# PBozmarov/RL-Environment-for-Component-Placement

Measured on AMD Instinct MI355X. Metric: env_steps_per_sec, higher is better.
Workload: dtype u64; 1 GPU; c3: 64x64 grid, 16 components, 48 pins, reward=centroid; envs_per_gpu=4096, queue_depth=2, instances=replay, fresh_instance_every_reset=False, incremental_obs=False, loop=fused, store_policy=sc1 (write-through)

## Files before the change

### rl-environment-for-component-placement_amd/csrc/pcb_device.h

```cpp
#pragma once
#include <hip/hip_runtime.h>
#include <math.h>
#include <stdint.h>

#include <type_traits>

#include "pcb_records.h"

__device__ inline u64 load_agent(const u64 *p) { return __hip_atomic_load(p, __ATOMIC_RELAXED, __HIP_MEMORY_SCOPE_AGENT); }
__device__ inline unsigned load_agent(const unsigned *p) { return __hip_atomic_load(p, __ATOMIC_RELAXED, __HIP_MEMORY_SCOPE_AGENT); }
__device__ inline int load_agent(const int *p) { return __hip_atomic_load(p, __ATOMIC_RELAXED, __HIP_MEMORY_SCOPE_AGENT); }
__device__ inline void store_agent(unsigned *p, unsigned v) { __hip_atomic_store(p, v, __ATOMIC_RELAXED, __HIP_MEMORY_SCOPE_AGENT); }
#ifdef PCBENV_STAMPS
#define STAMP(k) do { if ((threadIdx.x & (NT - 1)) == 0 && p.dbg) { unsigned long long t_; asm volatile("s_memtime %0\n\ts_waitcnt lgkmcnt(0)" : "=s"(t_) :: "memory"); p.dbg[(size_t)blockIdx.x * 32 + (k)] = t_; } } while (0)
#define STAMP_RT(k) do { if ((threadIdx.x & (NT - 1)) == 0 && p.dbg) { unsigned long long t_; asm volatile("s_memrealtime %0\n\ts_waitcnt lgkmcnt(0)" : "=s"(t_) :: "memory"); p.dbg[(size_t)blockIdx.x * 32 + (k)] = t_; } } while (0)
#define STAMP_T0() unsigned long long st0_; asm volatile("s_memtime %0\n\ts_waitcnt lgkmcnt(0)" : "=s"(st0_) :: "memory")
#define STAMP_ACC_SINCE(k, dep) do { unsigned long long t_; asm volatile("s_memtime %0\n\ts_waitcnt lgkmcnt(0)" : "=s"(t_) : "v"(dep) : "memory"); if ((threadIdx.x & (NT - 1)) == 0 && p.dbg) p.dbg[(size_t)blockIdx.x * 32 + (k)] += t_ - st0_; } while (0)
#define STAMP_ADD(k, v) do { if ((threadIdx.x & (NT - 1)) == 0 && p.dbg) p.dbg[(size_t)blockIdx.x * 32 + (k)] += (unsigned long long)(v); } while (0)
#define STAMP_ZERO(k) do { if ((threadIdx.x & (NT - 1)) == 0 && p.dbg) p.dbg[(size_t)blockIdx.x * 32 + (k)] = 0ull; } while (0)
#define STAMP_ROWS_BY_ENV(launch, e) DevParams p = (launch); if (p.dbg) p.dbg += ((long long)(e) - (long long)blockIdx.x) * 32
#else
#define STAMP(k) do { } while (0)
#define STAMP_RT(k) do { } while (0)
#define STAMP_T0() do { } while (0)
#define STAMP_ACC_SINCE(k, dep) do { } while (0)
#define STAMP_ADD(k, v) do { } while (0)
#define STAMP_ZERO(k) do { } while (0)
#define STAMP_ROWS_BY_ENV(launch, e) const DevParams &p = (launch)
#endif


template <int WW> struct Row;
template <> struct Row<1> {
    u64 a;
    __device__ static Row load(const u64 *p) { return Row{p[0]}; }
    __device__ void store(u64 *p) const { p[0] = a; }
    __device__ Row operator|(Row o) const { return Row{a | o.a}; }
    __device__ Row shr(int k) const { return Row{k >= 64 ? 0ull : a >> k}; }
    __device__ static Row zero() { return Row{0ull}; }
    __device__ bool any() const { return a != 0; }
    __device__ Row free_below(int n) const { return Row{n <= 0 ? 0ull : (~a & (n >= 64 ? ~0ull : ((1ull << n) - 1ull)))}; }
};
template <> struct Row<2> {
    u64 a, b;
    __device__ static Row load(const u64 *p) { return Row{p[0], p[1]}; }
    __device__ void store(u64 *p) const { p[0] = a; p[1] = b; }
    __device__ Row operator|(Row o) const { return Row{a | o.a, b | o.b}; }
    __device__ Row shr(int k) const {
        if (k == 0) return *this;
        if (k >= 128) return Row{0ull, 0ull};
        if (k >= 64) return Row{b >> (k - 64), 0ull};
        return Row{(a >> k) | (b << (64 - k)), b >> k};
    }
    __device__ static Row zero() { return Row{0ull, 0ull}; }
    __device__ bool any() const { return (a | b) != 0; }
    __device__ Row free_below(int n) const {
        u64 ma = n <= 0 ? 0ull : (n >= 64 ? ~0ull : ((1ull << n) - 1ull));
        u64 mb = n <= 64 ? 0ull : (n >= 128 ? ~0ull : ((1ull << (n - 64)) - 1ull));
        return Row{~a & ma, ~b & mb};
    }
};

template <int WW> __device__ inline Row<WW> hfold(Row<WW> r, int pw) {
    Row<WW> f = r;
    int s = 1;
    while (2 * s <= pw) { f = f | f.shr(s); s *= 2; }
    if (s < pw) f = f | f.shr(pw - s);
    return f;
}

typedef unsigned v4u __attribute__((ext_vector_type(4)));
#if defined(PCBENV_STORE_PLAIN)
struct ObsDst { unsigned char *base; };
__device__ inline ObsDst obs_dst(unsigned char *base, long long) { return ObsDst{base}; }
template <bool STREAM> __device__ inline void STORE16(const ObsDst &d, unsigned off, uint4 v) { *(uint4 *)(d.base + off) = v; }
#else
struct ObsDst { __amdgpu_buffer_rsrc_t rsrc; };
__device__ inline ObsDst obs_dst(unsigned char *base, long long bytes) {
    const uintptr_t b = (uintptr_t)base;
    const unsigned lo = (unsigned)__builtin_amdgcn_readfirstlane((int)(unsigned)b), hi = (unsigned)__builtin_amdgcn_readfirstlane((int)(unsigned)(b >> 32));
    unsigned char *ub = (unsigned char *)(((uintptr_t)hi << 32) | lo);
    return ObsDst{__builtin_amdgcn_make_buffer_rsrc(ub, 0, __builtin_amdgcn_readfirstlane((int)bytes), 0x00020000)};
}
#define PCBENV_AUX_SC1 16
#define PCBENV_AUX_NT 2
template <bool STREAM> __device__ inline void STORE16(const ObsDst &d, unsigned off, uint4 v) {
    const v4u w{v.x, v.y, v.z, v.w};
    __builtin_amdgcn_raw_buffer_store_b128(w, d.rsrc, (int)off, 0, STREAM ? (PCBENV_AUX_SC1 | PCBENV_AUX_NT) : PCBENV_AUX_SC1);
}
#endif

__device__ inline unsigned expand4(unsigned b) { return (b * 0x00204081u) & 0x01010101u; }
__device__ inline uint4 expand16(unsigned bits) {
    return make_uint4(expand4(bits & 15u), expand4((bits >> 4) & 15u), expand4((bits >> 8) & 15u), expand4((bits >> 12) & 15u));
}

__device__ inline void STORE16_dyn(const ObsDst &d, unsigned off, uint4 v, bool stream) { if (stream) STORE16<true>(d, off, v); else STORE16<false>(d, off, v); }
__device__ inline u64 lane_down(u64 a, int s, int lane) {
    const int src = (lane + s) << 2;
    const unsigned lo = (unsigned)__builtin_amdgcn_ds_bpermute(src, (int)(unsigned)a), hi = (unsigned)__builtin_amdgcn_ds_bpermute(src, (int)(unsigned)(a >> 32));
    return lane + s < WAVE ? (((u64)hi << 32) | lo) : 0ull;
}
template <int G> __device__ inline int group_inclusive_scan(int x, int lane) {
    const int row = lane & 15;
    int t;
    t = __builtin_amdgcn_update_dpp(0, x, 0x111, 0xF, 0xF, false); if (row >= 1) x += t;
    t = __builtin_amdgcn_update_dpp(0, x, 0x112, 0xF, 0xF, false); if (row >= 2) x += t;
    t = __builtin_amdgcn_update_dpp(0, x, 0x114, 0xF, 0xF, false); if (row >= 4) x += t;
    t = __builtin_amdgcn_update_dpp(0, x, 0x118, 0xF, 0xF, false); if (row >= 8) x += t;
    if (G >= 32) { t = __builtin_amdgcn_update_dpp(0, x, 0x142, 0xF, 0xF, false); if ((lane & 31) >= 16) x += t; }
    if (G == 64) { t = __builtin_amdgcn_update_dpp(0, x, 0x143, 0xF, 0xF, false); if (lane >= 32) x += t; }
// ... 9 lines not shown
```

### rl-environment-for-component-placement_amd/csrc/pcb_kernels.h

```cpp
#pragma once
#include "pcb_team.h"
#include "pcb_launch.h"

template <int KIND, int WW, int NW>
__global__ __launch_bounds__(64 * NW) void k_reset(DevParams p, const unsigned char *__restrict__ mask) {
    typedef Team<64 * NW> T;
    extern __shared__ __attribute__((aligned(16))) unsigned char smem[];
    const int e = xcd_contiguous_env((int)blockIdx.x, 0, p.B), lane = threadIdx.x;
    if (mask && !mask[e]) return;
    T::load_state(smem, p, e, lane);
    Lds l = carve(smem, p);
    const int row = out_row(p, p.slot, e);
    T::template reset_env<KIND, WW, true>(p, l, e, row, lane);
    if (lane == 0) {
        l.hdr->pre_action = 0u;
        l.hdr->term_seq = 0u;
        p.buf.reward[row] = 0.0;
        p.buf.done[row] = 0;
        if (p.buf.info) { p.buf.info[2 * (size_t)row] = nan(""); p.buf.info[2 * (size_t)row + 1] = nan(""); }
    }
    T::store_state(smem, p, e, lane);
}

template <int KIND, int WW, int NW>
__global__ __launch_bounds__(64 * NW) void k_gather(DevParams p, GatherArgs g) {
    typedef Team<64 * NW> T;
    extern __shared__ __attribute__((aligned(16))) unsigned char smem[];
    const int e = xcd_contiguous_env((int)blockIdx.x, 0, p.B), lane = threadIdx.x;
    const int j = __builtin_amdgcn_readfirstlane(g.src_index[e]);
    const bool take = (unsigned)j < (unsigned)g.src_B;
    if (!take && j != -1 && g.errors && lane == 0) atomicOr(g.errors, 1u);
    const unsigned char *own = p.state + (size_t)e * p.stateStride;
    T::load_state_from(smem, take ? g.src_state + (size_t)j * p.stateStride : own, p, lane);
    Lds l = carve(smem, p);
    if (take) {
        if (lane == 0) {
            const EnvHdr *oh = (const EnvHdr *)own;
            l.hdr->qcursor = oh->qcursor; l.hdr->episode = oh->episode;
            l.hdr->term_seq = 0u; l.hdr->term_pos = 0u;
            l.hdr->pre_action = 0u;
            if (KIND == PCBENV_PIN || KIND == PCBENV_SPATIAL) l.hdr->feat_gen = p.bind_gen;
        }
        T::lds_sync();
        const int row = out_row(p, p.slot, e);
        if (KIND == PCBENV_SPATIAL) T::build_pin_tables(p, l, lane);
        T::template emit_features_full<KIND>(p, l, row, lane);
        if (KIND == PCBENV_SPATIAL) {
            T::emit_component_grid(p, l, row, lane);
            T::feat_cache_fill(p, l, e, lane);
            T::lds_sync();
        }
        T::template mask_and_emit<KIND, WW>(p, l, row, lane, true, 0, p.H);
        if (KIND == PCBENV_SPATIAL) T::template emit_pin_grid<WW>(p, l, row, lane, 0, p.H);
        if (lane == 0) {
            p.buf.reward[row] = g.reward[j];
            p.buf.done[row] = g.done[j];
            if (p.buf.info) {
                p.buf.info[2 * (size_t)row] = g.info ? g.info[2 * (size_t)j] : nan("");
                p.buf.info[2 * (size_t)row + 1] = g.info ? g.info[2 * (size_t)j + 1] : nan("");
            }
        }
    }
    T::store_state(smem, p, e, lane);
}

template <int KIND, int WW, int NW, bool ROUTES, int BUILD, int GEO = STEP_GEO_RUNTIME>
__global__ __attribute__((amdgpu_waves_per_eu(4, 8))) __launch_bounds__(64 * NW) void k_step(DevParams p, int *__restrict__ actions, int fmt, int sampled,
                                               u64 seed, u64 first_env, u64 step_index, int num_steps_) {
    extern __shared__ __attribute__((aligned(16))) unsigned char smem[];
    constexpr bool TRAJ = BUILD == STEP_BUILD_SLOT || BUILD == STEP_BUILD_ROLLOUT;
    if (!TRAJ) p.stream_stores = BUILD == STEP_BUILD_INPLACE_STREAM;
    if (GEO == STEP_GEO_64) {
        static_assert(GEO == STEP_GEO_RUNTIME || (pcb_layout::is_pin_kind(KIND) && WW == 1 && NW == 1 && !ROUTES && !TRAJ), "pcb_layout::fixed_geometry_applies");
        constexpr pcb_layout::FixedGeometry g = pcb_layout::fixed_geometry(KIND);
        p.H = g.H; p.W = g.W; p.O = g.O; p.WW = g.WW;
        p.offOcc = g.offOcc; p.offVm = g.offVm; p.offComps = g.offComps;
        p.buf.grid = (uint8_t *)((uintptr_t)p.buf.grid & ~(uintptr_t)15);
        p.buf.action_mask = (uint8_t *)((uintptr_t)p.buf.action_mask & ~(uintptr_t)15);
        p.buf.pin_grid = (uint8_t *)((uintptr_t)p.buf.pin_grid & ~(uintptr_t)15);
    }
    const int num_steps = BUILD == STEP_BUILD_ROLLOUT ? num_steps_ : 1;
    __builtin_amdgcn_s_setprio(3);
    constexpr bool HELPERS = KIND == PCBENV_PIN || KIND == PCBENV_SPATIAL;
    const int nh = HELPERS ? p.term_wgs * p.term_hpe : 0;
    int e = (int)blockIdx.x - nh, role = ROLE_ENV, part = 0;
    if (e >= 0) e = xcd_contiguous_env((int)blockIdx.x, nh, p.B);
    unsigned pos = 0u;
    if (HELPERS && e < 0) {
        const unsigned hb = blockIdx.x, hpe = (unsigned)p.term_hpe, k = hb / hpe;
        part = (int)(hb - k * hpe);
        const unsigned ring = p.seq & 3u, cps = (unsigned)p.term_cap / TERM_SHARDS, shard = k & (TERM_SHARDS - 1u), idx = k >> TERM_SHARD_BITS;
        const unsigned cnt = (unsigned)__builtin_amdgcn_readfirstlane((int)load_agent(p.term_cnt + (ring * TERM_SHARDS + shard) * TERM_CNT_STRIDE));
        if (idx >= cps || idx >= cnt) return;
        pos = k;
        e = __builtin_amdgcn_readfirstlane(p.term_list[ring * (unsigned)p.term_cap + pos]);
        if ((unsigned)e >= (unsigned)p.B) return;
        role = part < REWARD_PARTS ? ROLE_REWARD : ROLE_FEATURES;
    } else if (p.term_cap > 0 && e == 0 && threadIdx.x < TERM_SHARDS) {
        unsigned *hist = p.term_cnt + TERM_HIST_OFFSET;
        unsigned longest = load_agent(p.term_cnt + (((p.seq & 3u) * TERM_SHARDS + threadIdx.x) * TERM_CNT_STRIDE));
        const unsigned h1 = hist[(p.seq + 1u) & 3u], h2 = hist[(p.seq + 2u) & 3u], h3 = hist[(p.seq + 3u) & 3u], told = hist[4];
        for (int o = TERM_SHARDS / 2; o > 0; o >>= 1) longest = max(longest, (unsigned)__shfl_xor((int)longest, o, TERM_SHARDS));
        const unsigned least = min(min(longest, h1), min(h2, h3));
        store_agent(p.term_cnt + ((((p.seq + 2u) & 3u) * TERM_SHARDS + threadIdx.x) * TERM_CNT_STRIDE), 0u);
        if (threadIdx.x == 0) {
            hist[p.seq & 3u] = longest;
            if (least > told || least + (told >> 3) + 2u < told) {
                hist[4] = least;
                __hip_atomic_store(p.term_seen, least, __ATOMIC_RELAXED, __HIP_MEMORY_SCOPE_SYSTEM);
            }
        }
    }
    Team<64 * NW>::template run_env<KIND, WW, ROUTES, TRAJ>(p, smem, e, threadIdx.x, actions, fmt, sampled, seed, first_env, step_index,
                                                           num_steps, role, part, pos);
}
```

### rl-environment-for-component-placement_amd/csrc/pcb_observe.h

```cpp
static __device__ inline void load_state_from(unsigned char *smem, const unsigned char *block, const DevParams &p, int lane) {
    const uint4 *src = (const uint4 *)block;
    uint4 *dst = (uint4 *)smem;
    const int n = (int)(p.stateStride / 16);
    if (n <= NT) {
        if (lane < n) dst[lane] = src[lane];
    } else {
        uint4 t[4];
        #pragma unroll
        for (int k = 0; k < 4; k++) { const int i = lane + k * NT; t[k] = i < n ? src[i] : make_uint4(0, 0, 0, 0); }
        #pragma unroll
        for (int k = 0; k < 4; k++) { const int i = lane + k * NT; if (i < n) dst[i] = t[k]; }
        for (int i = lane + 4 * NT; i < n; i += NT) dst[i] = src[i];
    }
    lds_sync();
}
static __device__ inline void load_state(unsigned char *smem, const DevParams &p, int e, int lane) {
    load_state_from(smem, p.state + (size_t)e * p.stateStride, p, lane);
}
static __device__ inline void store_state(const unsigned char *smem, const DevParams &p, int e, int lane) {
    lds_sync();
    uint4 *dst = (uint4 *)(p.state_out + (size_t)e * p.stateStride);
    const uint4 *src = (const uint4 *)smem;
    for (int i = lane; i < (int)(p.stateStride / 16); i += NT) dst[i] = src[i];
}

template <int KIND, int WW> static __device__ inline void emit_marginals(const DevParams &p, Lds &l, int row, int lane) {
    if (!p.buf.mask_rows && !p.buf.mask_orientation) return;
    const int H = p.H, plane = H * WW, O = p.O;
    for (int i = lane; i < O * H; i += NT) {
        const int o = i / H, r = i - o * H;
        const u64 *bits = l.vm + (o & 1) * plane + r * WW;
        bool a = false;
        for (int w = 0; w < WW; w++) a |= bits[w] != 0;
        if (p.buf.mask_rows) p.buf.mask_rows[(size_t)row * O * H + i] = a ? 1 : 0;
    }
    if (p.buf.mask_orientation) {
        for (int o = (int)(lane / WAVE); o < O; o += NT / WAVE) {
            bool a = false;
            for (int i = (lane & 63); i < plane; i += WAVE) a |= l.vm[(o & 1) * plane + i] != 0;
            a = __any(a);
            if ((lane & 63) == 0) p.buf.mask_orientation[(size_t)row * O + o] = a ? 1 : 0;
        }
    }
}

template <int KIND, int WW>
static __device__ inline bool mask_and_emit(const DevParams &p, Lds &l, int row, int lane, bool emit, int gr0, int gr1) {
    const int H = p.H, W = p.W, HW = H * W, plane = H * WW;
    const int cur = l.hdr->cur;
    unsigned char *m = (emit && p.buf.action_mask) ? p.buf.action_mask + (size_t)row * p.O * HW : 0;
    if (emit && p.buf.grid) emit_plane<WW>(p.buf.grid + (size_t)row * HW, l.occ, gr0, gr1, W, lane, p.stream_stores);
    bool any = false;
    if (KIND == PCBENV_SQUARE) {
        any = window_mask<WW>(l.occ, l.hf, l.vm, H, W, p.component_n, p.component_n, lane, &l.hdr->flag);
        if (m) emit_plane<WW>(m, l.vm, 0, H, W, lane, p.stream_stores);
        if (emit) emit_marginals<KIND, WW>(p, l, row, lane);
        return any;
    }
    const bool four = (KIND == PCBENV_PIN || KIND == PCBENV_SPATIAL);
    if (cur >= 0) {
        const int h = l.comps[cur].h, w = l.comps[cur].w;
        any = window_mask<WW>(l.occ, l.hf, l.vm, H, W, h, w, lane, &l.hdr->flag);
        if (m) { if (four) emit_plane2<WW>(m, m + 2 * HW, l.vm, H, W, lane, p.stream_stores); else emit_plane<WW>(m, l.vm, 0, H, W, lane, p.stream_stores); }
        if (h == w) {
            for (int i = lane; i < plane; i += NT) l.vm[plane + i] = l.vm[i];
            lds_sync();
        } else {
            any |= window_mask<WW>(l.occ, l.hf, l.vm + plane, H, W, w, h, lane, &l.hdr->flag);
        }
    } else {
        for (int i = lane; i < 2 * plane; i += NT) l.vm[i] = 0ull;
        lds_sync();
        if (m) { if (four) emit_plane2<WW>(m, m + 2 * HW, l.vm, H, W, lane, p.stream_stores); else emit_plane<WW>(m, l.vm, 0, H, W, lane, p.stream_stores); }
    }
    if (m) { if (four) emit_plane2<WW>(m + HW, m + 3 * HW, l.vm + plane, H, W, lane, p.stream_stores); else emit_plane<WW>(m + HW, l.vm + plane, 0, H, W, lane, p.stream_stores); }
    if (emit) emit_marginals<KIND, WW>(p, l, row, lane);
    return any;
}

#define CLS_EMPTY 0x80u
template <int WW> static __device__ inline void emit_pin_grid(const DevParams &p, Lds &l, int row, int lane, int r0, int r1) {
    if (!p.buf.pin_grid) return;
    const int W = p.W, HW = p.H * W, K = p.K;
    const int c0 = r0 * W, c1 = r1 * W;
    unsigned char *dst = p.buf.pin_grid + (size_t)row * HW * K;
    const long long b0 = (long long)c0 * K, b1 = (long long)c1 * K;
    if ((W & 15) == 0) {
        const int sh = (W & (W - 1)) == 0 ? __ffs(W) - 1 : -1;
        for (int ch = c0 / 16 + lane; ch < c1 / 16; ch += NT) {
            const int cell = ch * 16, r = sh >= 0 ? cell >> sh : cell / W, c = cell - r * W;
            uint4 v = expand16((unsigned)(l.occ[r * WW + (c >> 6)] >> (c & 63)) & 0xFFFFu);
            v.x |= (v.x ^ 0x01010101u) << 7; v.y |= (v.y ^ 0x01010101u) << 7; v.z |= (v.z ^ 0x01010101u) << 7; v.w |= (v.w ^ 0x01010101u) << 7;
            *(uint4 *)(l.cls + cell) = v;
        }
    } else {
        for (int i = c0 + lane; i < c1; i += NT) {
            int r = i / W, c = i - r * W;
            l.cls[i] = (unsigned char)(((l.occ[r * WW + (c >> 6)] >> (c & 63)) & 1ull) ? 1u : CLS_EMPTY);
        }
    }
    lds_sync();
    for (int q = lane; q < l.hdr->npins; q += NT) {
        const PinRec pr = l.pins[q];
        if (pr.abs_x >= r0 && pr.abs_x < r1 && pr.abs_y >= 0) l.cls[pr.abs_x * W + pr.abs_y] = (unsigned char)(pr.net + 2);
    }
    lds_sync();
    if ((b0 & 15) == 0 && (b1 & 15) == 0 && (((uintptr_t)dst) & 15) == 0) {
        const ObsDst d = obs_dst(dst, b1);
        const int first = ((int)(b0 / 16) + lane) * 16, dcell = 16 * NT / K, drem = 16 * NT - dcell * K;
        auto chunks = [&](auto stream_tag, auto cells_tag) {
            constexpr int NC = decltype(cells_tag)::value;
            int cell0 = first / K, rem = first - cell0 * K;
            for (int c = (int)(b0 / 16) + lane; c < (int)(b1 / 16); c += NT) {
                const int bb = c * 16;
                int cell = cell0;
                const int rem_now = rem;
                cell0 += dcell; rem += drem;
                if (rem >= K) { rem -= K; cell0++; }
                unsigned ones = 0u;
                if (K >= 5) {
                    unsigned cl[NC];
                    #pragma unroll
                    for (int j = 0; j < NC; j++) cl[j] = cell + j < c1 ? (unsigned)l.cls[cell + j] : CLS_EMPTY;
                    const int rel = -rem_now - 1;
                    #pragma unroll
                    for (int j = 0; j < NC; j++) {
                        const unsigned off = (unsigned)(rel + j * K + (int)cl[j]);
                        ones |= off < 16u ? 1u << off : 0u;
                    }
                } else {
                    for (int base = bb - rem_now; base < bb + 16 && cell < c1; base += K, cell++) {
                        const unsigned off = (unsigned)(base + (int)l.cls[cell] - 1 - bb);
                        if (off < 16u) ones |= 1u << off;
                    }
// ... 205 lines not shown
            double v = 0.0;
            if (c < nc) {
                const CompRec cr = l.comps[c];
                if (k == 0) v = cr.h; else if (k == 1) v = cr.w; else if (k == 2) v = cr.px; else if (k == 3) v = cr.py;
                else if (k == 4) v = (double)(cr.h * cr.w) / p.area;
                else {
                    const unsigned id = KIND == PCBENV_SPATIAL ? t.pid[c * p.mp + k - 5] : 0xFFFFu;
                    v = id == 0xFFFFu ? -1.0 : (double)id;
                }
            }
            cf[i] = v;
            c += dc; k += dk;
            if (k >= p.F) { k -= p.F; c++; }
        }
    }
    if (p.buf.placement_mask) {
        double *pm = p.buf.placement_mask + (size_t)row * p.C;
        for (int c = lane; c < p.C; c += NT) {
            const bool placed = c < nc && l.comps[c].px >= 0;
            pm[c] = KIND == PCBENV_RECT ? (placed ? 1.0 : 0.0) : (c >= nc ? 0.0 : placed ? 2.0 : c == cur ? 3.0 : 1.0);
        }
    }
    if (KIND == PCBENV_RECT && p.buf.component_mask) {
        double *cm = p.buf.component_mask + (size_t)row * p.C;
        for (int c = lane; c < p.C; c += NT) cm[c] = c < nc ? 1.0 : 0.0;
    }
    if (KIND == PCBENV_PIN || KIND == PCBENV_SPATIAL) {
        double *fn = p.buf.all_pins_num_feature ? p.buf.all_pins_num_feature + (size_t)row * p.pinRows * 4 : 0;
        double *fc = p.buf.all_pins_cat_feature ? p.buf.all_pins_cat_feature + (size_t)row * p.pinRows * p.catW : 0;
        if (!fn && !fc) return;
        if (KIND == PCBENV_SPATIAL) {
            for (int r = np + lane; r < p.pinRows; r += NT) {
                if (fn) { fn[4 * r] = 0.0; fn[4 * r + 1] = 0.0; fn[4 * r + 2] = 0.0; fn[4 * r + 3] = 0.0; }
                if (fc) { const double v = r == p.pinRows - 1 ? -1.0 : 0.0; fc[2 * r] = v; fc[2 * r + 1] = v; }
            }
            for (int q = lane; q < np; q += NT) {
                const PinRec pr = l.pins[q];
                const int r = pr.id & PIN_ID_MASK;
                if (fn) { fn[4 * r] = pr.rel_x; fn[4 * r + 1] = pr.rel_y; fn[4 * r + 2] = pr.abs_x; fn[4 * r + 3] = pr.abs_y; }
                if (fc) { fc[2 * r] = pr.net; fc[2 * r + 1] = pr.comp; }
            }
        } else if (p.pinRows <= p.ldsHfWords * 64) {
            u64 *rowbits = l.hf;
            lds_sync();
            for (int i = lane; i < p.ldsHfWords; i += NT) rowbits[i] = 0ull;
            lds_sync();
            for (int q = lane; q < np; q += NT) {
                const PinRec pr = l.pins[q];
                const int r = pr.comp * p.mp + (pr.id & PIN_ID_MASK);
                atomicOr((unsigned long long *)&rowbits[r >> 6], 1ull << (r & 63));
            }
            lds_sync();
            for (int r = lane; r < p.pinRows; r += NT) {
                if ((rowbits[r >> 6] >> (r & 63)) & 1ull) continue;
                if (fn) { fn[4 * r] = 0.0; fn[4 * r + 1] = 0.0; fn[4 * r + 2] = 0.0; fn[4 * r + 3] = 0.0; }
                if (fc) fc[r] = 0.0;
            }
            for (int q = lane; q < np; q += NT) {
                const PinRec pr = l.pins[q];
                if (pr.id & PIN_LOSER) continue;
                const int r = pr.comp * p.mp + (pr.id & PIN_ID_MASK);
                if (fn) { fn[4 * r] = pr.rel_x; fn[4 * r + 1] = pr.rel_y; fn[4 * r + 2] = pr.abs_x; fn[4 * r + 3] = pr.abs_y; }
                if (fc) fc[r] = pr.net;
            }
            lds_sync();
        } else {
            for (int i = lane; i < p.pinRows * 4; i += NT) if (fn) fn[i] = 0.0;
            for (int i = lane; i < p.pinRows; i += NT) if (fc) fc[i] = 0.0;
            store_drain_sync();
            for (int q = lane; q < np; q += NT) {
                const PinRec pr = l.pins[q];
                if (pr.id & PIN_LOSER) continue;
                const int r = pr.comp * p.mp + (pr.id & PIN_ID_MASK);
                if (fn) { fn[4 * r] = pr.rel_x; fn[4 * r + 1] = pr.rel_y; fn[4 * r + 2] = pr.abs_x; fn[4 * r + 3] = pr.abs_y; }
                if (fc) fc[r] = pr.net;
            }
        }
    }
}

template <int KIND, bool ROUTES>
static __device__ __forceinline__ void terminal_reward(const DevParams &p, Lds &l, int row, int lane, int part, int nparts, unsigned pos) {
    const bool placed_all = l.hdr->cur < 0;
    double reward, wl, ni;
    if (!placed_all) {
        reward = -p.w_wl * (p.max_wl / p.wl_norm) - p.w_int * (p.max_int / p.int_norm);
        wl = p.max_wl; ni = p.max_int;
    } else {
        double wsum[2] = {0.0, 0.0}; int cnt[2] = {0, 0};
        if (!ROUTES) route_centroid(p, l.hdr, l.pins, l.seg, lane, part, nparts, &wsum[0], &cnt[0]);
        else route_beam_or_both(p, l.hdr, l.pins, l.seg, lane, part, nparts, wsum, cnt);
        if (nparts > 1) {
            if (lane != 0) return;
            static_assert(REWARD_PARTS < 256 && PCBENV_MAX_PINS * (PCBENV_MAX_PINS - 1) / 2 < (1 << 28), "`mine`: 8 bits of arrivals, 28 bits per count of segment pairs");
            const u64 mine = 1ull | ((u64)(unsigned)cnt[0] << 8) | ((u64)(unsigned)cnt[1] << 36);
            const u64 before = atomicAdd((unsigned long long *)(p.term_arrive + pos), (unsigned long long)mine);
            if ((int)(before & 0xFFull) != nparts - 1) return;
            const u64 total = before + mine;
            cnt[0] = (int)((total >> 8) & 0xFFFFFFFull); cnt[1] = (int)(total >> 36);
            __hip_atomic_store(p.term_arrive + pos, 0ull, __ATOMIC_RELAXED, __HIP_MEMORY_SCOPE_AGENT);
        }
        const int pick = (ROUTES && p.reward_type == PCBENV_REWARD_BOTH && cnt[1] < cnt[0]) ? 1 : 0;
        wl = wsum[pick] / p.wl_norm;
        ni = (double)cnt[pick] / p.int_norm;
        reward = -1 * (p.w_wl * wl + p.w_int * ni);
    }
    if (lane == 0) {
        p.buf.reward[row] = reward;
        if (p.buf.info) { p.buf.info[2 * (size_t)row] = wl; p.buf.info[2 * (size_t)row + 1] = ni; }
    }
}
```

### rl-environment-for-component-placement_amd/csrc/pcb_reset.h

```cpp
static __device__ inline void fetch_instance(const DevParams &p, unsigned qcursor, int e, int lane, InstRegs &ir) {
    const unsigned slot = qcursor % (unsigned)p.Q;
    const unsigned char *rec = p.queue + ((size_t)slot * p.B + e) * p.instStride;
    const int *ih = (const int *)rec;
    const u64 *crec = (const u64 *)(rec + 16), *prec = crec + p.C;
    ir.nc = load_agent(ih); ir.nn = load_agent(ih + 1); ir.np = load_agent(ih + 2);
    ir.comp = lane < p.C ? load_agent(crec + lane) : 0ull;
    #pragma unroll
    for (int r = 0; r < 4; r++) { const int q = lane + r * NT; ir.pin[r] = q < p.P ? load_agent(prec + q) : 0ull; }
}

#define RESET_STATE_MASKS 1
#define RESET_FEATURES 2
#define RESET_ALL 3
template <int KIND, int WW, bool TRAJ> static __device__ inline void reset_env(const DevParams &p, Lds &l, int e, int row, int lane, int what = RESET_ALL) {
    const int H = p.H, W = p.W, HW = H * W;
    const bool owner = what & RESET_STATE_MASKS, feats = what & RESET_FEATURES;
    const bool full = TRAJ && p.num_slots > 1;
    lds_sync();
    InstRegs ir;
    if (KIND != PCBENV_SQUARE) {
        fetch_instance(p, l.hdr->qcursor, e, lane, ir);
        if (owner && p.gen_produced && lane == 0 && load_agent(p.gen_produced + e) <= l.hdr->qcursor) atomicOr(p.gen_errors, 1u);
    }
    bool rows_cleared = false;
    if (feats && (KIND == PCBENV_PIN || KIND == PCBENV_SPATIAL) && !full && l.hdr->feat_gen == p.bind_gen &&
        (KIND == PCBENV_SPATIAL || p.C * p.mp <= p.ldsHfWords * 64)) {
        u64 *rowbits = l.hf;
        if (KIND == PCBENV_PIN) {
            for (int i = lane; i < p.ldsHfWords; i += NT) rowbits[i] = 0ull;
            lds_sync();
            #pragma unroll
            for (int r = 0; r < 4; r++) {
                const int q = lane + r * NT;
                if (q < ir.np && q < p.P) {
                    const u64 w = ir.pin[r];
                    const int prow = (int)((w >> 24) & 0xFF) * p.mp + (int)((w >> 32) & PIN_ID_MASK);
                    atomicOr((unsigned long long *)&rowbits[prow >> 6], 1ull << (prow & 63));
                }
            }
            lds_sync();
        }
        for (int q = lane; q < l.hdr->npins; q += NT) {
            const PinRec pr = l.pins[q];
            const int prow = KIND == PCBENV_SPATIAL ? (pr.id & PIN_ID_MASK) : pr.comp * p.mp + (pr.id & PIN_ID_MASK);
            if (KIND == PCBENV_SPATIAL ? prow < ir.np : (int)((rowbits[prow >> 6] >> (prow & 63)) & 1ull)) continue;
            if (p.buf.all_pins_num_feature) {
                double *f = p.buf.all_pins_num_feature + ((size_t)row * p.pinRows + prow) * 4;
                f[0] = 0.0; f[1] = 0.0; f[2] = 0.0; f[3] = 0.0;
            }
            if (p.buf.all_pins_cat_feature) {
                double *f = p.buf.all_pins_cat_feature + ((size_t)row * p.pinRows + prow) * p.catW;
                f[0] = 0.0; if (KIND == PCBENV_SPATIAL) f[1] = 0.0;
            }
        }
        rows_cleared = true;
    }
    lds_sync();
    for (int i = lane; i < H * WW; i += NT) l.occ[i] = 0ull;
    if (KIND != PCBENV_SQUARE) {
        const int nc = ir.nc, nn = ir.nn, np = ir.np;
        if (lane < p.C) {
            const u64 w = ir.comp;
            CompRec cr; cr.h = (unsigned char)w; cr.w = (unsigned char)(w >> 8); cr.px = -1; cr.py = -1;
            cr.o = 0; cr.pad[0] = cr.pad[1] = cr.pad[2] = 0;
            if (lane >= nc) { cr.h = 0; cr.w = 0; }
            l.comps[lane] = cr;
        }
        #pragma unroll
        for (int r = 0; r < 4; r++) {
            const int q = lane + r * NT;
            if (q >= p.P) break;
            const u64 w = ir.pin[r];
            PinRec pr; pr.rel_x = (unsigned char)w; pr.rel_y = (unsigned char)(w >> 8); pr.abs_x = -1; pr.abs_y = -1;
            pr.net = (unsigned char)(w >> 16); pr.comp = (unsigned char)(w >> 24);
            pr.id = (unsigned short)(w >> 32);
            if (q >= np) { pr.rel_x = pr.rel_y = 0; pr.net = 0xFF; pr.comp = 0xFF; pr.id = 0; }
            l.pins[q] = pr;
        }
        if (lane == 0) {
            l.hdr->ncomp = (short)nc; l.hdr->nnets = (short)nn; l.hdr->npins = (short)np; l.hdr->cur = 0;
            l.hdr->qcursor += 1; l.hdr->episode += 1;
        }
        lds_sync();
        if (owner && lane == 0) store_agent(p.cursor_pub + e, l.hdr->qcursor);
        if (KIND == PCBENV_PIN && lane < WAVE) {
            if (np <= WAVE) {
                const unsigned key = lane < np ? ((unsigned)l.pins[lane].comp << 16) | (l.pins[lane].id & PIN_ID_MASK) : 0xFFFFFFFFu;
                u64 remaining = __ballot(lane < np);
                bool lose = false;
                while (remaining) {
                    const unsigned k = (unsigned)__builtin_amdgcn_readlane((int)key, __ffsll((long long)remaining) - 1);
                    const u64 m = __ballot(key == k);
                    if (key == k && lane != 63 - __clzll((long long)m)) lose = true;
                    remaining &= ~m;
                }
                if (lose) l.pins[lane].id |= PIN_LOSER;
            } else {
                unsigned key[4]; bool lose[4];
                #pragma unroll
                for (int r = 0; r < 4; r++) {
                    const int sidx = 64 * r + lane;
                    key[r] = sidx < np ? ((unsigned)l.pins[sidx].comp << 16) | (l.pins[sidx].id & PIN_ID_MASK) : 0xFFFFFFFFu;
                    lose[r] = false;
                }
                #pragma unroll
                for (int ri = 0; ri < 4; ri++) {
                    if (64 * ri >= np) break;
                    const int lim = min(64, np - 64 * ri);
                    for (int il = 0; il < lim; il++) {
                        const unsigned ki = (unsigned)__builtin_amdgcn_readlane((int)key[ri], il);
                        const int i = 64 * ri + il;
                        #pragma unroll
                        for (int r = 0; r < 4; r++)
                            if (64 * r < np && 64 * r + lane < i && key[r] == ki) lose[r] = true;
                    }
                }
                #pragma unroll
                for (int r = 0; r < 4; r++) if (lose[r]) l.pins[64 * r + lane].id |= PIN_LOSER;
            }
        }
    } else if (lane == 0) {
        l.hdr->ncomp = 0; l.hdr->nnets = 0; l.hdr->npins = 0; l.hdr->cur = 0; l.hdr->episode += 1;
    }
    lds_sync();
    STAMP(16);
    if (owner) mask_and_emit<KIND, WW>(p, l, row, lane, true, 0, H);
    STAMP(17);

    if (KIND != PCBENV_SQUARE) {
        const int nc = l.hdr->ncomp, np = l.hdr->npins;
        if (KIND == PCBENV_SPATIAL) {
            if (np <= WAVE) {
                if (lane < WAVE) {
                    const int comp = lane < np ? (int)l.pins[lane].comp : -1;
                    int rank = 0;
                    for (int c = 0; c < nc; c++) {
                        const u64 m = __ballot(comp == c);
                        if (comp == c) rank = __popcll(m & ((1ull << lane) - 1ull));
                    }
                    if (lane < np) l.rank[lane] = (unsigned char)rank;
                }
            } else {
                for (int q = lane; q < np; q += NT) {
                    const int comp = l.pins[q].comp;
                    int rank = 0;
                    #pragma unroll 4
                    for (int q2 = 0; q2 < np; q2++) rank += (q2 < q) & (l.pins[q2].comp == comp);
                    l.rank[q] = (unsigned char)rank;
                }
            }
            if (feats) build_pin_tables(p, l, lane);
        }
        if ((KIND == PCBENV_PIN || KIND == PCBENV_SPATIAL) && lane == 0) l.hdr->feat_gen = p.bind_gen;
        if (!feats) {
        } else if (full) {
            emit_features_full<KIND>(p, l, row, lane);
        } else {
            const PinTables t = pin_tables(p, l);
            if (p.buf.all_components_feature) {
                double *cf = p.buf.all_components_feature + (size_t)row * p.C * p.F;
                int c = lane / p.F, k = lane - c * p.F;
                const int dc = NT / p.F, dk = NT - dc * p.F;
                for (int i = lane; i < p.C * p.F; i += NT) {
                    double v = 0.0;
                    if (c < nc) {
                        const CompRec cr = l.comps[c];
                        if (k == 0) v = cr.h; else if (k == 1) v = cr.w; else if (k == 2 || k == 3) v = -1.0;
                        else if (k == 4) v = (double)(cr.h * cr.w) / p.area;
                        else {
                            const unsigned id = KIND == PCBENV_SPATIAL ? t.pid[c * p.mp + k - 5] : 0xFFFFu;
                            v = id == 0xFFFFu ? -1.0 : (double)id;
                        }
                    }
                    cf[i] = v;
                    c += dc; k += dk;
                    if (k >= p.F) { k -= p.F; c++; }
                }
            }
            STAMP(18);
            if (p.buf.placement_mask) {
                double *pm = p.buf.placement_mask + (size_t)row * p.C;
                for (int c = lane; c < p.C; c += NT)
                    pm[c] = KIND == PCBENV_RECT ? 0.0 : (c == 0 ? 3.0 : (c < nc ? 1.0 : 0.0));
            }
            if (KIND == PCBENV_RECT && p.buf.component_mask) {
                double *cm = p.buf.component_mask + (size_t)row * p.C;
                for (int c = lane; c < p.C; c += NT) cm[c] = c < nc ? 1.0 : 0.0;
            }
            if (KIND == PCBENV_PIN || KIND == PCBENV_SPATIAL) {
                if (!rows_cleared && p.buf.all_pins_num_feature) {
                    double *f = p.buf.all_pins_num_feature + (size_t)row * p.pinRows * 4;
                    for (int i = lane; i < p.pinRows * 4; i += NT) f[i] = 0.0;
                }
                if (!rows_cleared && p.buf.all_pins_cat_feature) {
                    double *f = p.buf.all_pins_cat_feature + (size_t)row * p.pinRows * p.catW;
                    for (int i = lane; i < p.pinRows * p.catW; i += NT)
                        f[i] = (KIND == PCBENV_SPATIAL && i >= (p.pinRows - 1) * p.catW) ? -1.0 : 0.0;
                }
                if (!rows_cleared) {
                    store_drain_sync();
                    __threadfence_block();
                }
                for (int q = lane; q < np; q += NT) {
                    const PinRec pr = l.pins[q];
                    write_pin_num<KIND>(p, row, pr);
                    if (p.buf.all_pins_cat_feature) {
                        if (KIND == PCBENV_SPATIAL) {
                            double *f = p.buf.all_pins_cat_feature + ((size_t)row * p.pinRows + (pr.id & PIN_ID_MASK)) * 2;
                            f[0] = pr.net; f[1] = pr.comp;
                        } else if (!(pr.id & PIN_LOSER)) {
                            p.buf.all_pins_cat_feature[(size_t)row * p.pinRows + pr.comp * p.mp + (pr.id & PIN_ID_MASK)] = pr.net;
                        }
                    }
                }
            }
        }
        STAMP(19);
        if (KIND == PCBENV_SPATIAL && feats) {
            if (p.buf.pin_grid) emit_zero(p.buf.pin_grid + (size_t)row * HW * p.K, (long long)HW * p.K, lane, p.stream_stores);
            emit_component_grid(p, l, row, lane);
            if (full) feat_cache_fill(p, l, e, lane);
        }
    }
    lds_sync();
}
```

### rl-environment-for-component-placement_amd/csrc/pcb_step.h

```cpp
static __device__ inline void presample_next(const DevParams &p, Lds &l, int sampled, int genv, u64 seed, u64 next_step, int lane) {
    if (lane >= WAVE) return;
#ifdef PCBENV_NO_PRESAMPLE
    sampled = 0;
#endif
    if (!sampled) { if (lane == 0) l.hdr->pre_action = 0u; return; }
    int o, x, y;
    sample_action(l.vm, p, genv, lane, seed, next_step, &o, &x, &y);
    if (lane == 0) {
        l.hdr->pre_seed = seed; l.hdr->pre_step = next_step; l.hdr->pre_genv = (unsigned)genv;
        l.hdr->pre_action = (unsigned)o | ((unsigned)x << 8) | ((unsigned)y << 16) | 0x80000000u;
    }
}

static __device__ __forceinline__ void draw_action(const DevParams &p, Lds &l, int genv, int lane, u64 seed, u64 step, int *o, int *x, int *y) {
    if (lane < WAVE) {
        sample_action(l.vm, p, genv, lane, seed, step, o, x, y);
        if (NT > WAVE && lane == 0) { l.hdr->pad[0] = (unsigned)*o; l.hdr->pad[1] = (unsigned)*x; l.hdr->flag = (unsigned)*y; }
    }
    if (NT > WAVE) {
        lds_sync();
        *o = (int)l.hdr->pad[0]; *x = (int)l.hdr->pad[1]; *y = (int)l.hdr->flag;
    }
}

// ... 97 lines not shown
        if (KIND == PCBENV_SPATIAL) emit_pin_grid<WW>(p, l, row, lane, 0, H);
    }
    if (mode != MODE_REWARD) {
        if (lane == 0) p.buf.done[row] = done ? 1 : 0;
        if (KIND == PCBENV_SQUARE || KIND == PCBENV_RECT) { if (lane == 0) p.buf.reward[row] = valid ? 1.0 : 0.0; }
        else if (!done) { if (lane == 0) p.buf.reward[row] = 0.0; }
    }
    if ((KIND == PCBENV_PIN || KIND == PCBENV_SPATIAL) && done && !helpers_route)
        terminal_reward<KIND, ROUTES>(p, l, row, lane, part, mode == MODE_REWARD ? REWARD_PARTS : 1, pos);
    STAMP(9);
    if (done && auto_reset && mode != MODE_REWARD) {
        store_drain_sync();
        reset_env<KIND, WW, TRAJ>(p, l, e, row, lane, mode == MODE_DELEGATED ? RESET_STATE_MASKS : RESET_ALL);
    }
    STAMP(10);
}

#define ROLE_ENV 0
#define ROLE_REWARD 1
#define ROLE_FEATURES 2
template <int KIND, int WW, bool ROUTES, bool TRAJ>
static __device__ __forceinline__ void run_env(const DevParams &p_launch, unsigned char *smem, int e, int lane0, int *actions, int fmt, int sampled,
                                               u64 seed, u64 first_env, u64 step_index, int num_steps, int role, int part, unsigned pos) {
    STAMP_ROWS_BY_ENV(p_launch, role == ROLE_ENV ? e : p_launch.B + (int)pos * (REWARD_PARTS + 1) + part);
    const int H = p.H, W = p.W, HW = H * W;
    STAMP_RT(30);
    STAMP(0);
    load_state(smem, p, e, lane0);
    Lds l = carve(smem, p);
    STAMP(1);
    int mode = MODE_ALL;
    if (KIND != PCBENV_SQUARE && p.term_wgs > 0) {
        const u64 mk = ((u64)l.hdr->term_seq << 32) | l.hdr->term_pos;
        const bool listed = (unsigned)(mk >> 32) == p.seq && (unsigned)mk < (unsigned)p.term_wgs && (role == ROLE_ENV || (unsigned)mk == pos);
        const int cur = l.hdr->cur;
        const bool last = cur >= 0 && cur == l.hdr->ncomp - 1;
        if (listed && last) mode = role == ROLE_ENV ? MODE_DELEGATED : role == ROLE_REWARD ? MODE_REWARD : MODE_FEATURES;
        else if (role != ROLE_ENV) return;
    }
    const int genv = (int)first_env + e;
    const size_t per_step = (size_t)p.B * (fmt == PCBENV_ACTION_TUPLE ? 3 : 1);
    int slot = p.slot;
    for (int t = 0; t < num_steps; t++) {
        int lane = lane0;
        asm volatile("" : "+v"(lane));
        int o = 0, x = 0, y = 0;
        int *act = actions + per_step * (size_t)t;
        if (mode == MODE_FEATURES) {
        } else if (sampled) {
            const unsigned pa = l.hdr->pre_action, pg = l.hdr->pre_genv;
            const u64 ps = l.hdr->pre_seed, pst = l.hdr->pre_step;
            if ((t == 0) & (pa >> 31) & (ps == seed) & (pst == step_index) & (pg == (unsigned)genv)) {
                o = (int)(pa & 0xFFu); x = (int)((pa >> 8) & 0xFFu); y = (int)((pa >> 16) & 0xFFu);
                STAMP(21);
            } else {
                draw_action(p, l, genv, lane, seed, step_index + (u64)t, &o, &x, &y);
            }
            if (lane == 0 && role == ROLE_ENV) {
                if (fmt == PCBENV_ACTION_FLAT) act[e] = PCB_FLATTEN_ACTION(o, x, y, HW, W);
                else { act[3 * e] = o; act[3 * e + 1] = x; act[3 * e + 2] = y; }
            }
        } else if (fmt == PCBENV_ACTION_FLAT) {
            unflatten_action(act[e], p.O, HW, W, &o, &x, &y);
        } else {
            o = act[3 * e]; x = act[3 * e + 1]; y = act[3 * e + 2];
            if (KIND == PCBENV_SQUARE) o = 0;
        }
        STAMP(2);
        const unsigned episode = l.hdr->episode;
        transition<KIND, WW, ROUTES, TRAJ>(p, l, e, TRAJ ? out_row(p, slot, e) : e, lane, o, x, y, mode, part, pos);
        if (t + 1 < num_steps) {
            if (l.hdr->episode != episode) store_drain_sync(); else lds_sync();
            if (++slot == p.num_slots) slot = 0;
        }
    }
    if (mode == MODE_REWARD || mode == MODE_FEATURES) { STAMP(11); STAMP_RT(31); return; }
    presample_next(p, l, sampled && num_steps == 1, genv, seed, step_index + 1, lane0);
    if (KIND != PCBENV_SQUARE && p.term_cap > 0 && lane0 == 0) {
        const int cur = l.hdr->cur;
        u64 mark = 0ull;
        if (cur >= 0 && cur == l.hdr->ncomp - 1) {
            const unsigned ring = (p.seq + 1u) & 3u, cps = (unsigned)p.term_cap / TERM_SHARDS;
            const unsigned shard = ((unsigned)e * 0x9E3779B1u) >> (32 - TERM_SHARD_BITS);
            const unsigned idx = atomicAdd(p.term_cnt + (ring * TERM_SHARDS + shard) * TERM_CNT_STRIDE, 1u);
            if (idx < cps) {
                const unsigned mpos = idx * TERM_SHARDS + shard;
                p.term_list[ring * (unsigned)p.term_cap + mpos] = e;
                mark = ((u64)(p.seq + 1u) << 32) | mpos;
            }
        }
        l.hdr->term_seq = (unsigned)(mark >> 32); l.hdr->term_pos = (unsigned)mark;
    }
    STAMP(20);
    store_state(smem, p, e, lane0);
    STAMP(11);
    STAMP_RT(31);
}
```

### rl-environment-for-component-placement_amd/csrc/pcb_team_io.h

```cpp
static __device__ inline void lds_sync() {
    __builtin_amdgcn_fence(__ATOMIC_RELEASE, "workgroup", "local");
    if (NT > WAVE) __builtin_amdgcn_s_barrier(); else __builtin_amdgcn_wave_barrier();
    __builtin_amdgcn_fence(__ATOMIC_ACQUIRE, "workgroup", "local");
}
static __device__ inline void store_drain_sync() {
    asm volatile("s_waitcnt vmcnt(0)" ::: "memory");
    lds_sync();
}
static __device__ inline bool block_any(bool v, unsigned *flag) {
    if (NT == WAVE) return __any(v);
    if (threadIdx.x == 0) *flag = 0;
    lds_sync();
    if (__any(v) && (threadIdx.x & 63) == 0) *flag = 1;
    lds_sync();
    return *flag != 0;
}

template <int WW, bool STREAM> static __device__ inline void emit_plane_(unsigned char *dst, const u64 *bits, int r0, int r1, int W, int lane) {
    if ((W & 15) == 0 && (((uintptr_t)dst) & 15) == 0) {
        const ObsDst d = obs_dst(dst, (long long)r1 * W);
        const int sh = (W & (W - 1)) == 0 ? __ffs(W) - 1 : -1;
        for (int c = r0 * W / 16 + lane; c < r1 * W / 16; c += NT) {
            int cell = c * 16, r = sh >= 0 ? cell >> sh : cell / W, col = cell - r * W;
            unsigned b = (unsigned)(bits[r * WW + (col >> 6)] >> (col & 63)) & 0xFFFFu;
            STORE16<STREAM>(d, (unsigned)cell, expand16(b));
        }
    } else {
        for (int i = r0 * W + lane; i < r1 * W; i += NT) {
            int r = i / W, col = i - r * W;
            dst[i] = (unsigned char)((bits[r * WW + (col >> 6)] >> (col & 63)) & 1ull);
        }
    }
}
template <bool STREAM> static __device__ inline void emit_zero_(unsigned char *dst, long long bytes, int lane) {
    if ((bytes & 15) == 0 && (((uintptr_t)dst) & 15) == 0) {
        const ObsDst d = obs_dst(dst, bytes);
        for (int c = lane; c < (int)(bytes / 16); c += NT) STORE16<STREAM>(d, (unsigned)c * 16u, make_uint4(0, 0, 0, 0));
    } else {
        for (long long i = lane; i < bytes; i += NT) dst[i] = 0;
    }
}
template <int WW, bool STREAM> static __device__ inline void emit_plane2_(unsigned char *dst, unsigned char *dst2, const u64 *bits, int H, int W, int lane) {
    if ((W & 15) == 0 && (((uintptr_t)dst) & 15) == 0 && (((uintptr_t)dst2) & 15) == 0) {
        const ObsDst d = obs_dst(dst, (long long)H * W), d2 = obs_dst(dst2, (long long)H * W);
        const int sh = (W & (W - 1)) == 0 ? __ffs(W) - 1 : -1;
        if (__builtin_constant_p(H * W) && __builtin_constant_p(W) && (H * W / 16) % NT == 0 && H * W / 16 / NT <= 8) {
            PCB_UNROLL
            for (int k = 0; k < H * W / 16 / NT; k++) {
                const int cell = (lane + k * NT) * 16, r = sh >= 0 ? cell >> sh : cell / W, col = cell - r * W;
                unsigned b = (unsigned)(bits[r * WW + (col >> 6)] >> (col & 63)) & 0xFFFFu;
                const uint4 v = expand16(b);
                STORE16<STREAM>(d, (unsigned)cell, v);
                STORE16<STREAM>(d2, (unsigned)cell, v);
            }
            return;
        }
        for (int c = lane; c < H * W / 16; c += NT) {
            int cell = c * 16, r = sh >= 0 ? cell >> sh : cell / W, col = cell - r * W;
            unsigned b = (unsigned)(bits[r * WW + (col >> 6)] >> (col & 63)) & 0xFFFFu;
            const uint4 v = expand16(b);
            STORE16<STREAM>(d, (unsigned)cell, v);
            STORE16<STREAM>(d2, (unsigned)cell, v);
        }
    } else {
        emit_plane_<WW, STREAM>(dst, bits, 0, H, W, lane);
        emit_plane_<WW, STREAM>(dst2, bits, 0, H, W, lane);
    }
}
template <int WW> static __device__ inline void emit_plane(unsigned char *dst, const u64 *bits, int r0, int r1, int W, int lane, bool stream) {
    if (stream) emit_plane_<WW, true>(dst, bits, r0, r1, W, lane); else emit_plane_<WW, false>(dst, bits, r0, r1, W, lane);
}
template <int WW> static __device__ inline void emit_plane2(unsigned char *dst, unsigned char *dst2, const u64 *bits, int H, int W, int lane, bool stream) {
    if (stream) emit_plane2_<WW, true>(dst, dst2, bits, H, W, lane); else emit_plane2_<WW, false>(dst, dst2, bits, H, W, lane);
}
static __device__ inline void emit_zero(unsigned char *dst, long long bytes, int lane, bool stream) {
    if (stream) emit_zero_<true>(dst, bytes, lane); else emit_zero_<false>(dst, bytes, lane);
}

template <int WW>
static __device__ inline bool window_mask(const u64 *occ, u64 *hf, u64 *vm, int H, int W, int ph, int pw, int lane, unsigned *flag) {
    if (pcb_layout::fold_across_lanes(WW, NT, H)) {
        u64 a = lane < H ? hfold<1>(Row<1>::load(occ + lane), pw).a : 0ull;
        int s = 1;
        while (2 * s <= ph) { a |= lane_down(a, s, lane); s *= 2; }
        if (s < ph) a |= lane_down(a, ph - s, lane);
        const u64 v = (lane + ph <= H) ? Row<1>{a}.free_below(W - pw + 1).a : 0ull;
        if (lane < H) vm[lane] = v;
        return __any(v != 0ull);
    }
    for (int r = lane; r < H; r += NT) hfold<WW>(Row<WW>::load(occ + r * WW), pw).store(hf + r * WW);
    lds_sync();
    bool any = false;
    for (int r = lane; r < H; r += NT) {
        Row<WW> v = Row<WW>::zero();
        if (r + ph <= H) {
            Row<WW> acc = Row<WW>::load(hf + r * WW);
            for (int k = 1; k < ph; k++) acc = acc | Row<WW>::load(hf + (r + k) * WW);
            v = acc.free_below(W - pw + 1);
        }
        v.store(vm + r * WW);
        any |= v.any();
    }
    return block_any(any, flag);
}
// ... 1 lines not shown
```

Baseline: 227.0 million env-steps/s.

## Prefetch kernarg lines and load cold params at use in fixed-geometry build

For the PCB_PART==4 build, the step kernel first issues one scalar load per 64-byte line of the kernarg segment to warm the constant cache. Rarely used DevParams fields (reward weights, queue pointers, terminal lists) are then read from the kernarg segment at their point of use, so they are not held in SGPRs for the whole kernel. When the grid size is a compile-time constant and incremental obs is off, the grid plane is emitted with a fully unrolled store loop. The goal is lower scalar-register pressure and less kernel-entry latency, at the cost of extra scalar loads and a build-specific code path.

```diff
diff --git a/rl-environment-for-component-placement_amd/csrc/pcb_device.h b/rl-environment-for-component-placement_amd/csrc/pcb_device.h
--- a/rl-environment-for-component-placement_amd/csrc/pcb_device.h
+++ b/rl-environment-for-component-placement_amd/csrc/pcb_device.h
@@ -27,6 +27,31 @@
 #define STAMP_ADD(k, v) do { } while (0)
 #define STAMP_ZERO(k) do { } while (0)
 #define STAMP_ROWS_BY_ENV(launch, e) const DevParams &p = (launch)
+#endif
+
+#if defined(PCB_PART) && PCB_PART == 4
+#define PCB_GEO64_UNIT 1
+template <class T> __device__ __forceinline__ T kernarg_field_at_use(unsigned offset) {
+    typedef const __attribute__((address_space(4))) unsigned char *kernarg_ptr;
+    kernarg_ptr k = (kernarg_ptr)__builtin_amdgcn_kernarg_segment_ptr();
+    asm volatile("" : "+s"(k));
+    return *(const __attribute__((address_space(4))) T *)(k + offset);
+}
+template <int BYTES> __device__ __forceinline__ void kernarg_warm() {
+    static_assert(BYTES > 0x200 + 4 && BYTES <= 0x240, "one load per 64-byte line of the segment, and its last word");
+    typedef const __attribute__((address_space(4))) unsigned char *kernarg_ptr;
+    kernarg_ptr k = (kernarg_ptr)__builtin_amdgcn_kernarg_segment_ptr();
+    unsigned t0, t1, t2, t3, t4, t5, t6, t7, t8, t9;
+    asm volatile("s_load_dword %0, %10, 0x0\n\ts_load_dword %1, %10, 0x40\n\ts_load_dword %2, %10, 0x80\n\ts_load_dword %3, %10, 0xc0\n\t"
+                 "s_load_dword %4, %10, 0x100\n\ts_load_dword %5, %10, 0x140\n\ts_load_dword %6, %10, 0x180\n\ts_load_dword %7, %10, 0x1c0\n\t"
+                 "s_load_dword %8, %10, 0x200\n\ts_load_dword %9, %10, %11\n\ts_waitcnt lgkmcnt(0)"
+                 : "=&s"(t0), "=&s"(t1), "=&s"(t2), "=&s"(t3), "=&s"(t4), "=&s"(t5), "=&s"(t6), "=&s"(t7), "=&s"(t8), "=&s"(t9)
+                 : "s"(k), "n"((BYTES - 4) & ~3));
+}
+#define PCB_COLD(p, field) kernarg_field_at_use<std::remove_cv_t<std::remove_reference_t<decltype((p).field)>>>((unsigned)offsetof(DevParams, field))
+#else
+#define PCB_GEO64_UNIT 0
+#define PCB_COLD(p, field) ((p).field)
 #endif
 
 
diff --git a/rl-environment-for-component-placement_amd/csrc/pcb_kernels.h b/rl-environment-for-component-placement_amd/csrc/pcb_kernels.h
--- a/rl-environment-for-component-placement_amd/csrc/pcb_kernels.h
+++ b/rl-environment-for-component-placement_amd/csrc/pcb_kernels.h
@@ -69,6 +69,9 @@
                                                u64 seed, u64 first_env, u64 step_index, int num_steps_) {
     extern __shared__ __attribute__((aligned(16))) unsigned char smem[];
     constexpr bool TRAJ = BUILD == STEP_BUILD_SLOT || BUILD == STEP_BUILD_ROLLOUT;
+#if PCB_GEO64_UNIT
+    kernarg_warm<sizeof(DevParams) + sizeof(int *) + 2 * sizeof(int) + 3 * sizeof(u64) + sizeof(int)>();
+#endif
     if (!TRAJ) p.stream_stores = BUILD == STEP_BUILD_INPLACE_STREAM;
     if (GEO == STEP_GEO_64) {
         static_assert(GEO == STEP_GEO_RUNTIME || (pcb_layout::is_pin_kind(KIND) && WW == 1 && NW == 1 && !ROUTES && !TRAJ), "pcb_layout::fixed_geometry_applies");
diff --git a/rl-environment-for-component-placement_amd/csrc/pcb_observe.h b/rl-environment-for-component-placement_amd/csrc/pcb_observe.h
--- a/rl-environment-for-component-placement_amd/csrc/pcb_observe.h
+++ b/rl-environment-for-component-placement_amd/csrc/pcb_observe.h
@@ -49,7 +49,10 @@
     const int H = p.H, W = p.W, HW = H * W, plane = H * WW;
     const int cur = l.hdr->cur;
     unsigned char *m = (emit && p.buf.action_mask) ? p.buf.action_mask + (size_t)row * p.O * HW : 0;
-    if (emit && p.buf.grid) emit_plane<WW>(p.buf.grid + (size_t)row * HW, l.occ, gr0, gr1, W, lane, p.stream_stores);
+    if (emit && p.buf.grid) {
+        if (PCB_GEO64_UNIT && __builtin_constant_p(HW) && !(p.flags & PCBENV_FLAG_INCREMENTAL_OBS)) emit_plane<WW>(p.buf.grid + (size_t)row * HW, l.occ, 0, H, W, lane, p.stream_stores);
+        else emit_plane<WW>(p.buf.grid + (size_t)row * HW, l.occ, gr0, gr1, W, lane, p.stream_stores);
+    }
     bool any = false;
     if (KIND == PCBENV_SQUARE) {
         any = window_mask<WW>(l.occ, l.hf, l.vm, H, W, p.component_n, p.component_n, lane, &l.hdr->flag);
@@ -421,10 +424,12 @@
 template <int KIND, bool ROUTES>
 static __device__ __forceinline__ void terminal_reward(const DevParams &p, Lds &l, int row, int lane, int part, int nparts, unsigned pos) {
     const bool placed_all = l.hdr->cur < 0;
+    const double w_wl = PCB_COLD(p, w_wl), w_int = PCB_COLD(p, w_int), wl_norm = PCB_COLD(p, wl_norm), int_norm = PCB_COLD(p, int_norm);
     double reward, wl, ni;
     if (!placed_all) {
-        reward = -p.w_wl * (p.max_wl / p.wl_norm) - p.w_int * (p.max_int / p.int_norm);
-        wl = p.max_wl; ni = p.max_int;
+        const double max_wl = PCB_COLD(p, max_wl), max_int = PCB_COLD(p, max_int);
+        reward = -w_wl * (max_wl / wl_norm) - w_int * (max_int / int_norm);
+        wl = max_wl; ni = max_int;
     } else {
         double wsum[2] = {0.0, 0.0}; int cnt[2] = {0, 0};
         if (!ROUTES) route_centroid(p, l.hdr, l.pins, l.seg, lane, part, nparts, &wsum[0], &cnt[0]);
@@ -433,16 +438,17 @@
             if (lane != 0) return;
             static_assert(REWARD_PARTS < 256 && PCBENV_MAX_PINS * (PCBENV_MAX_PINS - 1) / 2 < (1 << 28), "`mine`: 8 bits of arrivals, 28 bits per count of segment pairs");
             const u64 mine = 1ull | ((u64)(unsigned)cnt[0] << 8) | ((u64)(unsigned)cnt[1] << 36);
-            const u64 before = atomicAdd((unsigned long long *)(p.term_arrive + pos), (unsigned long long)mine);
+            u64 *arrive = PCB_COLD(p, term_arrive) + pos;
+            const u64 before = atomicAdd((unsigned long long *)arrive, (unsigned long long)mine);
             if ((int)(before & 0xFFull) != nparts - 1) return;
             const u64 total = before + mine;
             cnt[0] = (int)((total >> 8) & 0xFFFFFFFull); cnt[1] = (int)(total >> 36);
-            __hip_atomic_store(p.term_arrive + pos, 0ull, __ATOMIC_RELAXED, __HIP_MEMORY_SCOPE_AGENT);
+            __hip_atomic_store(arrive, 0ull, __ATOMIC_RELAXED, __HIP_MEMORY_SCOPE_AGENT);
         }
         const int pick = (ROUTES && p.reward_type == PCBENV_REWARD_BOTH && cnt[1] < cnt[0]) ? 1 : 0;
-        wl = wsum[pick] / p.wl_norm;
-        ni = (double)cnt[pick] / p.int_norm;
-        reward = -1 * (p.w_wl * wl + p.w_int * ni);
+        wl = wsum[pick] / wl_norm;
+        ni = (double)cnt[pick] / int_norm;
+        reward = -1 * (w_wl * wl + w_int * ni);
     }
     if (lane == 0) {
         p.buf.reward[row] = reward;
diff --git a/rl-environment-for-component-placement_amd/csrc/pcb_reset.h b/rl-environment-for-component-placement_amd/csrc/pcb_reset.h
--- a/rl-environment-for-component-placement_amd/csrc/pcb_reset.h
+++ b/rl-environment-for-component-placement_amd/csrc/pcb_reset.h
@@ -1,6 +1,6 @@
 static __device__ inline void fetch_instance(const DevParams &p, unsigned qcursor, int e, int lane, InstRegs &ir) {
-    const unsigned slot = qcursor % (unsigned)p.Q;
-    const unsigned char *rec = p.queue + ((size_t)slot * p.B + e) * p.instStride;
+    const unsigned slot = qcursor % (unsigned)PCB_COLD(p, Q);
+    const unsigned char *rec = PCB_COLD(p, queue) + ((size_t)slot * p.B + e) * PCB_COLD(p, instStride);
     const int *ih = (const int *)rec;
     const u64 *crec = (const u64 *)(rec + 16), *prec = crec + p.C;
     ir.nc = load_agent(ih); ir.nn = load_agent(ih + 1); ir.np = load_agent(ih + 2);
@@ -20,7 +20,8 @@
     InstRegs ir;
     if (KIND != PCBENV_SQUARE) {
         fetch_instance(p, l.hdr->qcursor, e, lane, ir);
-        if (owner && p.gen_produced && lane == 0 && load_agent(p.gen_produced + e) <= l.hdr->qcursor) atomicOr(p.gen_errors, 1u);
+        const unsigned *produced = PCB_COLD(p, gen_produced);
+        if (owner && produced && lane == 0 && load_agent(produced + e) <= l.hdr->qcursor) atomicOr(PCB_COLD(p, gen_errors), 1u);
     }
     bool rows_cleared = false;
     if (feats && (KIND == PCBENV_PIN || KIND == PCBENV_SPATIAL) && !full && l.hdr->feat_gen == p.bind_gen &&
@@ -82,7 +83,7 @@
             l.hdr->qcursor += 1; l.hdr->episode += 1;
         }
         lds_sync();
-        if (owner && lane == 0) store_agent(p.cursor_pub + e, l.hdr->qcursor);
+        if (owner && lane == 0) store_agent(PCB_COLD(p, cursor_pub) + e, l.hdr->qcursor);
         if (KIND == PCBENV_PIN && lane < WAVE) {
             if (np <= WAVE) {
                 const unsigned key = lane < np ? ((unsigned)l.pins[lane].comp << 16) | (l.pins[lane].id & PIN_ID_MASK) : 0xFFFFFFFFu;
@@ -159,6 +160,7 @@
             const PinTables t = pin_tables(p, l);
             if (p.buf.all_components_feature) {
                 double *cf = p.buf.all_components_feature + (size_t)row * p.C * p.F;
+                const double area = PCB_COLD(p, area);
                 int c = lane / p.F, k = lane - c * p.F;
                 const int dc = NT / p.F, dk = NT - dc * p.F;
                 for (int i = lane; i < p.C * p.F; i += NT) {
@@ -166,7 +168,7 @@
                     if (c < nc) {
                         const CompRec cr = l.comps[c];
                         if (k == 0) v = cr.h; else if (k == 1) v = cr.w; else if (k == 2 || k == 3) v = -1.0;
-                        else if (k == 4) v = (double)(cr.h * cr.w) / p.area;
+                        else if (k == 4) v = (double)(cr.h * cr.w) / area;
                         else {
                             const unsigned id = KIND == PCBENV_SPATIAL ? t.pid[c * p.mp + k - 5] : 0xFFFFu;
                             v = id == 0xFFFFu ? -1.0 : (double)id;
diff --git a/rl-environment-for-component-placement_amd/csrc/pcb_step.h b/rl-environment-for-component-placement_amd/csrc/pcb_step.h
--- a/rl-environment-for-component-placement_amd/csrc/pcb_step.h
+++ b/rl-environment-for-component-placement_amd/csrc/pcb_step.h
@@ -203,10 +203,10 @@
         if (cur >= 0 && cur == l.hdr->ncomp - 1) {
             const unsigned ring = (p.seq + 1u) & 3u, cps = (unsigned)p.term_cap / TERM_SHARDS;
             const unsigned shard = ((unsigned)e * 0x9E3779B1u) >> (32 - TERM_SHARD_BITS);
-            const unsigned idx = atomicAdd(p.term_cnt + (ring * TERM_SHARDS + shard) * TERM_CNT_STRIDE, 1u);
+            const unsigned idx = atomicAdd(PCB_COLD(p, term_cnt) + (ring * TERM_SHARDS + shard) * TERM_CNT_STRIDE, 1u);
             if (idx < cps) {
                 const unsigned mpos = idx * TERM_SHARDS + shard;
-                p.term_list[ring * (unsigned)p.term_cap + mpos] = e;
+                PCB_COLD(p, term_list)[ring * (unsigned)p.term_cap + mpos] = e;
                 mark = ((u64)(p.seq + 1u) << 32) | mpos;
             }
         }
diff --git a/rl-environment-for-component-placement_amd/csrc/pcb_team_io.h b/rl-environment-for-component-placement_amd/csrc/pcb_team_io.h
--- a/rl-environment-for-component-placement_amd/csrc/pcb_team_io.h
+++ b/rl-environment-for-component-placement_amd/csrc/pcb_team_io.h
@@ -20,6 +20,15 @@
     if ((W & 15) == 0 && (((uintptr_t)dst) & 15) == 0) {
         const ObsDst d = obs_dst(dst, (long long)r1 * W);
         const int sh = (W & (W - 1)) == 0 ? __ffs(W) - 1 : -1;
+        if (PCB_GEO64_UNIT && __builtin_constant_p(r0) && __builtin_constant_p(r1 * W) && r0 == 0 && (r1 * W / 16) % NT == 0 && r1 * W / 16 / NT <= 8) {
+            PCB_UNROLL
+            for (int k = 0; k < r1 * W / 16 / NT; k++) {
+                const int cell = (lane + k * NT) * 16, r = sh >= 0 ? cell >> sh : cell / W, col = cell - r * W;
+                unsigned b = (unsigned)(bits[r * WW + (col >> 6)] >> (col & 63)) & 0xFFFFu;
+                STORE16<STREAM>(d, (unsigned)cell, expand16(b));
+            }
+            return;
+        }
         for (int c = r0 * W / 16 + lane; c < r1 * W / 16; c += NT) {
             int cell = c * 16, r = sh >= 0 ? cell >> sh : cell / W, col = cell - r * W;
             unsigned b = (unsigned)(bits[r * WW + (col >> 6)] >> (col & 63)) & 0xFFFFu;
```

Result: faster. 232.3 million env-steps/s, median of 6 (+2.4%).
